# bibendovsky/oalsfxpp

Measured on AMD Instinct MI355X. Metric: Msamples/sec EAX reverb, 256-frame buffers, batch=4096; % HBM roofline, higher is better.
Workload: dtype f32

## Files before the change

oalsfxpp_amd/csrc/hip/reverb.hip:

```cpp
#include <float.h>

#include "common.hpp"
#include "wave_effects_body.hpp"

namespace oalsfx_hip {

namespace {

constexpr int kRow = 68;
constexpr int kGroups = 3;
constexpr int kSteadyGroups = 6;
constexpr int kRngFloats = OALSFX_RV_MAX_UPDATE;

namespace ut {
enum {
    TAP4 = 0,
    LO = 24,
    BMASK = 44,
    FEED4 = 49,
    CR_R = 50, CR_RF = 51,
    ECOEF = 52, ELCOEF = 56,
    MISC = 60,
    LPB = 64, HPB = 68,
    TL0 = 72, TL1 = 76, TH0 = 80, TH1 = 84,
// ... 558 lines not shown
        __hip_atomic_fetch_add(ctx.fault, 1u, __ATOMIC_RELAXED, __HIP_MEMORY_SCOPE_SYSTEM);
    }
    }
    stamp();
    const bool sf = SF && go && first && (flags & kFilterInside) != 0 && has_filter;
    float* const sfmisc = sh.sf_misc[SF ? wib : 0];
    auto sfrow = [&](int stage, int r) -> float* { return sh.sf_rows[SF ? wib : 0][SF ? stage * kSfRows + r : 0]; };
    if constexpr (SF) {
        if (lane == 0) sh.sf_all[wib] = sf ? 1 : 0;
        if (sf) {
            const oalsfx_source_params& SGp = ctx.source[inst];
            const oalsfx_source_state& SGs = ctx.source_state[inst];
            if (lane < 2) {
                const oalsfx_send_params& sp = lane == 0 ? SGp.direct : SGp.aux[slot];
                float* t = sfmisc + sfm::TAB + 12 * lane;
                t[0] = sp.lp.b0; t[1] = sp.lp.b1; t[2] = sp.lp.b2; t[3] = sp.hp.b0; t[4] = sp.hp.b1; t[5] = sp.hp.b2;
                t[6] = sp.lp.a1; t[7] = sp.lp.a2; t[8] = sp.hp.a1; t[9] = sp.hp.a2;
                const bool enabled = lane == 0 || sp.out_channels != 0;
                reinterpret_cast<int*>(t)[10] = enabled ? (((sp.filter_type & OALSFX_AF_LOW_PASS) ? 1 : 0) | ((sp.filter_type & OALSFX_AF_HIGH_PASS) ? 2 : 0) | 4) : 0;
            }
            if (lane < kSfRows) {
                const int sd = lane / CH, c = lane % CH, at = sd ? 1 + slot : 0;
                const oalsfx_hist_t lp = SGs.lp[at][c], hp = SGs.hp[at][c];
                float* h = sfmisc + sfm::HIST + 6 * lane;
                h[0] = lp.x[0]; h[1] = lp.x[1]; h[2] = lp.y[0]; h[3] = lp.y[1]; h[4] = hp.y[0]; h[5] = hp.y[1];
            }
        }
    }
    const bool filtered = !sf && (flags & kFiltered) != 0 && has_filter;
    const float* src = ctx.raw_src + static_cast<size_t>(inst) * ctx.io_stride;
    const float* wsrc = src;
    if (filtered) {
        src = ctx.src + static_cast<size_t>(inst) * ctx.src_stride;
        wsrc = ctx.wet_src + static_cast<size_t>(inst) * ctx.src_stride;
    }
    float* dst = ctx.dst + static_cast<size_t>(inst) * ctx.io_stride;
    float* mixbuf = ctx.mixbuf ? ctx.mixbuf + static_cast<size_t>(inst) * nch * OALSFX_MAX_CHUNK : nullptr;
    const float b2a = 0.288675134595F;

    v4f n_e = {0, 0, 0, 0}, n_a = n_e, n_el = n_e, n_lt = n_e, n_la = n_e, n_ll = n_e;
    float n_in0 = 0.0F, n_in1 = 0.0F;
    float n_inv[MC ? 8 : 1] = {};
    float n_w0 = 0.0F, n_w1 = 0.0F;
    float n_wv[MC ? 8 : 1] = {};
    auto tapbase = [&](int tile) -> int { return (XF && fc0 < OALSFX_RV_FADE_SAMPLES && fc0 + (tile << 6) >= OALSFX_RV_FADE_SAMPLES) ? kTapN : static_cast<int>(ut::TAP4); };
    auto load4 = [&](unsigned t4x, int group, auto ring, int base = ut::TAP4) -> v4f {
        constexpr int r = decltype(ring)::value;
        const v4u d = *reinterpret_cast<const v4u*>(utu + base + 4 * group);
        const v4u lo = *reinterpret_cast<const v4u*>(utu + ut::LO + 4 * r);
        const unsigned bm = utu[ut::BMASK + r];
        v4f v;
        v.x = ld_ring<r>(slab_b, ((t4x - d.x) & bm) | lo.x);
        v.y = ld_ring<r>(slab_b, ((t4x - d.y) & bm) | lo.y);
        v.z = ld_ring<r>(slab_b, ((t4x - d.z) & bm) | lo.z);
        v.w = ld_ring<r>(slab_b, ((t4x - d.w) & bm) | lo.w);
        return v;
    };
    constexpr bool AW = FP && !HY && !MD && !ST && !MC && !XF;
    v4f w_e = {0, 0, 0, 0}, w_el = w_e, w_lt = w_e, w_ll = w_e;
    auto load4w = [&](unsigned tile4, int group, auto ring) -> v4f {
        constexpr int r = decltype(ring)::value;
        const v4u d = *reinterpret_cast<const v4u*>(utu + ut::TAP4 + 4 * group);
        const v4u lo = *reinterpret_cast<const v4u*>(utu + ut::LO + 4 * r);
        const unsigned bm = utu[ut::BMASK + r];
        const unsigned l4 = 256u + 4u * static_cast<unsigned>(lane);
        v4f v;
        v.x = ld_ring<r>(slab_b, ((((tile4 - d.x) & ~255u) + l4) & bm) | lo.x);
        v.y = ld_ring<r>(slab_b, ((((tile4 - d.y) & ~255u) + l4) & bm) | lo.y);
        v.z = ld_ring<r>(slab_b, ((((tile4 - d.z) & ~255u) + l4) & bm) | lo.z);
        v.w = ld_ring<r>(slab_b, ((((tile4 - d.w) & ~255u) + l4) & bm) | lo.w);
        return v;
    };
    auto rotate4 = [&](const v4f& before, const v4f& last, unsigned tile4, int group) -> v4f {
        const v4u d = *reinterpret_cast<const v4u*>(utu + ut::TAP4 + 4 * group);
        auto one = [&](float b, float l, unsigned dj) -> float {
            const int k = static_cast<int>(((tile4 - dj) & 255u) >> 2);
            const float merged = lane >= k ? b : l;
            return __uint_as_float(static_cast<unsigned>(__builtin_amdgcn_ds_bpermute(((lane + k) & 63) << 2, static_cast<int>(__float_as_uint(merged)))));
        };
        v4f v;
        v.x = one(before.x, last.x, d.x); v.y = one(before.y, last.y, d.y); v.z = one(before.z, last.z, d.z); v.w = one(before.w, last.w, d.w);
        return v;
    };
    auto strow = [&](int k) -> float* { return utf + ut::SIZE + k * kRow; };
    float* modrow = utf + ut::SIZE;
    int mod_pos = v_modidx;
    auto next_mod_delays = [&](int samples_or_64) -> int {
        const int samples = RG ? samples_or_64 : 64;
        if (lane == 0) {
            float r = mod_f;
            const float depth = mod_depth, coeff = mod_coeff;
            for (int i = 0; i < samples; ++i) {
                r = lerpf(r, depth, coeff);
                modrow[i] = r;
            }
        }
        wave_sync();
        const float fv = modrow[lane];
        mod_f = modrow[samples - 1];
        wave_sync();
        int index;
        if (!RG && v_modrange >= 64) {
            index = mod_pos + lane;
            if (index >= v_modrange) index -= v_modrange;
            mod_pos += 64;
            if (mod_pos >= v_modrange) mod_pos -= v_modrange;
        } else {
            index = (mod_pos + lane) % v_modrange;
            mod_pos += 64;
        }
        const float sinus = glibc_sinf(6.28318530717958647692F * index / v_modrange);
        return lround_away(fv * sinus);
    };
    int md_next = 0, md_cur = 0;
    auto mb_buffer = [&](int pos) -> int {
        const int tile = __builtin_amdgcn_readfirstlane(pos) >> 6;
        return __builtin_amdgcn_readfirstlane(tile / (mbt->frames >> 6));
    };
    auto issue_input = [&](int posx) {
        const int px = min(posx, frames - 1);
        if (MC) {
#pragma unroll
            for (int c = 0; c < 8; ++c)
                if (c < nch) n_inv[MC ? c : 0] = src[static_cast<size_t>(px) * nch + c];
            if (filtered) {
#pragma unroll
                for (int c = 0; c < 8; ++c)
                    if (c < nch) n_wv[MC ? c : 0] = wsrc[static_cast<size_t>(px) * nch + c];
            }
        } else if (CH == 2) {
            const float2 v = *reinterpret_cast<const float2*>(src + static_cast<size_t>(px) * 2);
            n_in0 = v.x; n_in1 = v.y;
            if (filtered) {
                const float2 u = *reinterpret_cast<const float2*>(wsrc + static_cast<size_t>(px) * 2);
                n_w0 = u.x; n_w1 = u.y;
            }
        } else {
            n_in0 = src[px];
            if (filtered) n_w0 = wsrc[px];
        }
    };
    auto issue_taps_a = [&](unsigned t4x, int base) {
        if (AW) n_e = load4w(t4x - 4u * static_cast<unsigned>(lane), 0, RingId<OALSFX_RV_MAIN>{});
        else if (!HY || !(late_mask & 1u)) n_e = load4(t4x, 0, RingId<OALSFX_RV_MAIN>{}, base);
        if (!HY || !(late_mask & 2u)) n_a = load4(t4x, 1, RingId<OALSFX_RV_EARLY_AP>{}, base);
    };
    auto issue_taps_b = [&](unsigned t4x, int base) {
        if (AW) {
            const unsigned tile4 = t4x - 4u * static_cast<unsigned>(lane);
            n_el = load4w(tile4, 2, RingId<OALSFX_RV_EARLY_LINE>{});
            n_lt = load4w(tile4, 3, RingId<OALSFX_RV_MAIN>{});
            n_ll = load4w(tile4, 5, RingId<OALSFX_RV_LATE_LINE>{});
            return;
        }
        if (!HY || !(late_mask & 4u)) n_el = load4(t4x, 2, RingId<OALSFX_RV_EARLY_LINE>{}, base);
        if (!HY || !(late_mask & 8u)) n_lt = load4(t4x, 3, RingId<OALSFX_RV_MAIN>{}, base);
        if (!HY || !(late_mask & 32u)) n_ll = load4(MD ? t4x - 4u * static_cast<unsigned>(md_next) : t4x, 5, RingId<OALSFX_RV_LATE_LINE>{}, base);
    };
    auto issue_taps_c = [&](unsigned t4x, int base) {
        if (!HY || !(late_mask & 16u)) n_la = load4(t4x, 4, RingId<OALSFX_RV_LATE_AP>{}, base);
    };
    auto store4 = [&](unsigned p4, auto ring, float v0, float v1, float v2, float v3) {
        constexpr int r = decltype(ring)::value;
        const v4u lo = *reinterpret_cast<const v4u*>(utu + ut::LO + 4 * r);
        const unsigned wp = p4 & utu[ut::BMASK + r];
        st_ring<r>(slab_b, wp | lo.x, v0); st_ring<r>(slab_b, wp | lo.y, v1); st_ring<r>(slab_b, wp | lo.z, v2); st_ring<r>(slab_b, wp | lo.w, v3);
    };
    static_assert(CR == 0 || (AW && !SF), "line-aligned stores: the plain FP builds");
    auto cr_lane_before = [&](unsigned r) -> int { return ((lane - static_cast<int>(r)) & 63) << 2; };
    auto cr_rot = [&](int from4, float v) -> float { return __uint_as_float(static_cast<unsigned>(__builtin_amdgcn_ds_bpermute(from4, static_cast<int>(__float_as_uint(v))))); };
    auto carry_store = [&](unsigned tile4, auto ring, unsigned r, const v4f& rot, const v4f& before, bool head, bool tail, int L) {
        constexpr int rg = decltype(ring)::value;
        const v4u lo = *reinterpret_cast<const v4u*>(utu + ut::LO + 4 * rg);
        const unsigned bm = utu[ut::BMASK + rg];
        const bool held = lane < static_cast<int>(r);
        const int rl = static_cast<int>(r) + (RG ? L : 64);
        const unsigned at = tile4 - 4u * r + 4u * static_cast<unsigned>(lane);
        if (!(head && held) && (!RG || lane < rl)) {
            const unsigned wp = at & bm;
            st_ring<rg>(slab_b, wp | lo.x, held ? before.x : rot.x); st_ring<rg>(slab_b, wp | lo.y, held ? before.y : rot.y);
            st_ring<rg>(slab_b, wp | lo.z, held ? before.z : rot.z); st_ring<rg>(slab_b, wp | lo.w, held ? before.w : rot.w);
        }
        if (tail && (RG ? lane < rl - 64 : held)) {
            const unsigned wp = (at + 256u) & bm;
            st_ring<rg>(slab_b, wp | lo.x, rot.x); st_ring<rg>(slab_b, wp | lo.y, rot.y); st_ring<rg>(slab_b, wp | lo.z, rot.z); st_ring<rg>(slab_b, wp | lo.w, rot.w);
        }
    };
    auto cr_tail = [&](int site) -> v4f* { return reinterpret_cast<v4f*>(&sh.cr_tails[CR == 2 ? wib : 0][CR == 2 ? site : 0][lane & 31][0]); };
    auto carry_store_lds = [&](unsigned tile4, auto ring, int site, const v4f& rot, bool head, bool tail, int L) {
        v4f* t = cr_tail(site);
        const unsigned r = utu[ut::CR_R];
        const v4f before = *t;
        carry_store(tile4, ring, r, rot, before, head, tail, L);
        if (lane < static_cast<int>(r)) *t = rot;
    };
    v4f cr_feed = {0, 0, 0, 0};
    const int cw = (lane >> 2) & (NW - 1), cc = lane & 3;
    float* crowI0 = lds_all[cw] + (0 * 4 + cc) * kRow;
    float* crowI1 = lds_all[cw] + (1 * 4 + cc) * kRow;
    float* crowI2 = lds_all[cw] + (2 * 4 + cc) * kRow;
    float* crowL1 = lds_all[cw] + (4 * 4 + cc) * kRow;
    float* crowL2 = lds_all[cw] + (5 * 4 + cc) * kRow;
    float* cdat = chain_all[cw][cc];

    if (CR != 0 && go) {
        if (lane == 0) {
            utu[ut::CR_R] = static_cast<unsigned>(offset) & 31u;
            utu[ut::CR_RF] = (static_cast<unsigned>(offset) - (utu[ut::FEED4] >> 2)) & 31u;
        }
        wave_sync();
    }
    stamp();
    if (go) {
        if (FP && !(flags & kFiltered)) { n_in0 = early_in0; n_in1 = early_in1; }
        else issue_input(lane);
        if (AW) w_e = load4w((static_cast<unsigned>(offset) << 2) - 256u, 0, RingId<OALSFX_RV_MAIN>{});
        issue_taps_a(static_cast<unsigned>(offset + lane) << 2, tapbase(0));
    }
    stamp();
    lds_barrier();
    stamp();
    bool any_go = false;
    bool any_eax = false;
    bool any_sf = false;
#pragma unroll
    for (int k = 0; k < NW; ++k) { any_go |= go_all[k] != 0; any_eax |= eax_all[k] != 0; if (SF) any_sf |= sh.sf_all[k] != 0; }
    const bool chain_on = (lane < 4 * NW) && go_all[cw] != 0;
    const bool chain2_on = chain_on && eax_all[cw] != 0;
    const int duty = (wib - group) & (NW - 1);

    const int tiles = any_go ? (RG ? (frames + 63) >> 6 : frames >> 6) : 0;
    float o0 = 0.0F, o1 = 0.0F;
    float outv[MC ? 8 : 1] = {};
    int fc = fc0, blk_start = 0, blk_end = 0, blk_counter = 1;
    float g_step = 0.0F, g_run = 0.0F;
    bool g_ramp = false;
    unsigned long long ramp_mask = 0ULL;
    auto grow = [&](int q) -> float* { return q < 12 ? rowL(q >> 2, q & 3) + 4 : utf + ut::SIZE + (2 + q - 12) * kRow + 4; };
    constexpr bool EH = FP && !SF && !ST;
    auto hand_back = [&]() {
        if (go) {
            if (lane < 4) {
                const float* ch = chain_all[wib][lane];
                S.lp[lane].x[0] = ch[coop::LPX0]; S.lp[lane].x[1] = ch[coop::LPX1];
                S.lp[lane].y[0] = ch[coop::LPY0]; S.lp[lane].y[1] = ch[coop::LPY1];
                if (eax) {
                    S.hp[lane].x[0] = ch[coop::LPY0]; S.hp[lane].x[1] = ch[coop::LPY1];
                    S.hp[lane].y[0] = ch[coop::HPY0]; S.hp[lane].y[1] = ch[coop::HPY1];
                }
                S.t60[lane][0][0] = ch[coop::T60X]; S.t60[lane][0][1] = ch[coop::T60O1];
                S.t60[lane][1][0] = ch[coop::T60O1]; S.t60[lane][1][1] = ch[coop::T60O2];
            }
            if (lane == 0) {
                S.mod_index = static_cast<int>((static_cast<long long>(v_modidx) + frames) % v_modrange);
                S.offset = offset + frames;
                if (MD && mod_on) S.mod_filter = mod_f;
            }
            if (XF && xf_active) {
                if (q_valid) {
                    if (q_stage) S.late_cur_gain[q_line][q_chan] = g_cur;
                    else S.early_cur_gain[q_line][q_chan] = g_cur;
                }
                const bool fade_over = fc >= OALSFX_RV_FADE_SAMPLES;
                if (fc0 < OALSFX_RV_FADE_SAMPLES && fade_over && lane < 24) (&S.cur_early_tap[0])[lane] = static_cast<int32_t>(utu[kTapN + lane] >> 2);
                if (lane == 0) {
                    S.fade_count = fc;
                    S.mod_range = v_modrange;
                    SS.seen_seq = SP.update_seq;
                }
                if (ctx.exact) {
                    const unsigned level = gains_rest_level(q_valid, g_cur, g_tgt);
                    if (lane == 0) ctx.exact[sidx] = fade_over ? level : 0u;
                }
            }
            if (SF && sf) {
                if (lane < kSfRows) {
                    const int sd = lane / CH, c = lane % CH, at = sd ? 1 + slot : 0;
                    if (reinterpret_cast<const int*>(sfmisc + sfm::TAB + 12 * sd)[10] & 4) {
                        const float* h = sfmisc + sfm::HIST + 6 * lane;
                        oalsfx_source_state& SGs = ctx.source_state[inst];
                        oalsfx_hist_t lp, hp;
                        lp.x[0] = h[0]; lp.x[1] = h[1]; lp.y[0] = h[2]; lp.y[1] = h[3];
                        hp.x[0] = h[2]; hp.x[1] = h[3]; hp.y[0] = h[4]; hp.y[1] = h[5];
                        SGs.lp[at][c] = lp;
                        SGs.hp[at][c] = hp;
                    }
                }
            } else if (FP && !RG) {
                if (first && !filtered && lane < nch)
                    send_history_follow_values(ctx, inst, lane, send_mask, lane == 0 ? hist_new[0] : hist_new[CH - 1], lane == 0 ? hist_old[0] : hist_old[CH - 1]);
            } else if (first && !filtered && lane < nch) send_history_follow(ctx, inst, lane, nch, frames, src);
        }
        if constexpr (FP) {
            if (go) {
                if (lane == 0) {
                    miscu[hot::M_EPOCH] = epoch_now;
                    miscu[hot::M_OFFSET] = static_cast<unsigned>(offset + frames);
                    miscu[hot::M_MOD_F] = __float_as_uint(mod_f);
                    miscu[hot::M_MOD_INDEX] = static_cast<unsigned>((static_cast<long long>(v_modidx) + frames) % v_modrange);
                    miscu[hot::M_MOD_ON] = (MD && ((mod_depth != 0.0F) || (mod_f != 0.0F))) ? 1u : 0u;
                }
                wave_sync();
                v4u* rec = reinterpret_cast<v4u*>(ctx.hot + sidx * hot::SIZE);
                if (lane >= 48) rec[lane] = *reinterpret_cast<const v4u*>(miscu + 4 * (lane - 48));
                else if (lane >= 32) rec[lane] = *reinterpret_cast<const v4u*>(&chain_all[wib][0][0] + 4 * (lane - 32));
                else if (!hit) rec[lane] = *reinterpret_cast<const v4u*>(utu + 4 * lane);
            }
        }
    };
    for (int it = (SF && any_sf) ? -1 : 0; it <= tiles && tiles > 0; ++it) {
        const int ta = it, tb = it - 1, tc = it + 1;
        const bool has_a = ta >= 0 && ta < tiles, has_b = tb >= 0, has_c = SF && tc < tiles;
        const int pos_a = (ta << 6) + lane, pos_b = (tb << 6) + lane;
        const int La = RG ? min(64, frames - (ta << 6)) : 64;
        const int Lb = RG ? min(64, frames - (tb << 6)) : 64;
        const bool act = RG ? lane < Lb : true;
        const unsigned t4 = static_cast<unsigned>(offset + pos_b) << 2;
        const unsigned tile_b4 = static_cast<unsigned>(offset + (tb << 6)) << 2;
        const bool head_b = tb == 0, tail_b = tb == tiles - 1;
        float oa0 = 0.0F, oa1 = 0.0F;
        float outva[MC ? 8 : 1] = {};
        v4f p_e = n_e, p_a = n_a, p_el = n_el, p_lt = n_lt, p_la = n_la, p_ll = n_ll;
        if (AW && go && has_b) {
            const unsigned tile4 = static_cast<unsigned>(offset + (tb << 6)) << 2;
            p_e = rotate4(w_e, n_e, tile4, 0); p_el = rotate4(w_el, n_el, tile4, 2); p_lt = rotate4(w_lt, n_lt, tile4, 3); p_ll = rotate4(w_ll, n_ll, tile4, 5);
            w_e = n_e; w_el = n_el; w_lt = n_lt; w_ll = n_ll;
        }
        const int xg = eax ? 0 : 2;
        const bool xf_faded = XF && xf_active && has_b && fc0 + (tb << 6) < OALSFX_RV_FADE_SAMPLES;
        const float mu = static_cast<float>(fc0 + pos_b) * (1.0F / OALSFX_RV_FADE_SAMPLES);
        v4f q_e = {0, 0, 0, 0}, q_a = q_e, q_lt = q_e, q_el = q_e;
        auto mix4 = [&](v4f& a, const v4f& b) {
            a.x = lerpf(a.x, b.x, mu); a.y = lerpf(a.y, b.y, mu); a.z = lerpf(a.z, b.z, mu); a.w = lerpf(a.w, b.w, mu);
        };
        const int tb_base = tapbase(tb);

        if (go) {
            if (MD) {
                md_cur = md_next;
                if (mod_on && has_a) md_next = next_mod_delays(min(64, frames - (ta << 6)));
            }
            if (HY && has_b) {
                const int base = tapbase(tb);
                if (late_mask & 1u) p_e = load4(t4, 0, RingId<OALSFX_RV_MAIN>{}, base);
                if (late_mask & 2u) p_a = load4(t4, 1, RingId<OALSFX_RV_EARLY_AP>{}, base);
                if (late_mask & 4u) p_el = load4(t4, 2, RingId<OALSFX_RV_EARLY_LINE>{}, base);
                if (late_mask & 8u) p_lt = load4(t4, 3, RingId<OALSFX_RV_MAIN>{}, base);
                if (late_mask & 16u) p_la = load4(t4, 4, RingId<OALSFX_RV_LATE_AP>{}, base);
                if (late_mask & 32u) p_ll = load4(MD ? t4 - 4u * static_cast<unsigned>(md_cur) : t4, 5, RingId<OALSFX_RV_LATE_LINE>{}, base);
            }
            if (XF && xf_faded) {
                q_e = load4(t4, 0, RingId<OALSFX_RV_MAIN>{}, kTapN); q_a = load4(t4, 1, RingId<OALSFX_RV_EARLY_AP>{}, kTapN);
                q_lt = load4(t4, 3, RingId<OALSFX_RV_MAIN>{}, kTapN);
                q_el = load4(t4, 2, RingId<OALSFX_RV_EARLY_LINE>{}, kTapN);
                const v4f q_ll = load4(t4 - 4u * static_cast<unsigned>(md_cur), 5, RingId<OALSFX_RV_LATE_LINE>{}, kTapN);
                mix4(p_ll, q_ll);
            }
            if (has_a && it > 0) issue_taps_a(t4 + 256u, tapbase(ta));
            __builtin_amdgcn_sched_barrier(0);
        }
        v2f e01 = {0, 0}, e23 = {0, 0};
        float dg = 0.0F, ac = 0.0F, sx = 0.0F, sy = 0.0F;
        if (go && has_b) {
            if constexpr (CR == 2) {
                const int from = 4 + (cr_lane_before(utu[ut::CR_R]) >> 2);
                carry_store_lds(tile_b4, RingId<OALSFX_RV_MAIN>{}, 0, v4f{rowI(xg, 0)[from], rowI(xg, 1)[from], rowI(xg, 2)[from], rowI(xg, 3)[from]}, head_b, tail_b, Lb);
            } else if (act) store4(t4, RingId<OALSFX_RV_MAIN>{}, rowI(xg, 0)[4 + lane], rowI(xg, 1)[4 + lane], rowI(xg, 2)[4 + lane], rowI(xg, 3)[4 + lane]);
            wave_sync();
            const v4f misc = *reinterpret_cast<const v4f*>(utf + ut::MISC);
            dg = misc.x; ac = misc.y; sx = misc.z; sy = misc.w;
            const v4f ec = *reinterpret_cast<const v4f*>(utf + ut::ECOEF);
            const v4f elc = *reinterpret_cast<const v4f*>(utf + ut::ELCOEF);
            if (ST && (short_mask & 1u)) {
                auto hand_over = [&](v4f& v, int base) {
                    const v4u d = *reinterpret_cast<const v4u*>(utu + base);
                    const int e0 = static_cast<int>(d.x >> 2), e1 = static_cast<int>(d.y >> 2), e2 = static_cast<int>(d.z >> 2), e3 = static_cast<int>(d.w >> 2);
                    if (lane >= e0) v.x = rowI(xg, 0)[4 + lane - e0];
                    if (lane >= e1) v.y = rowI(xg, 1)[4 + lane - e1];
                    if (lane >= e2) v.z = rowI(xg, 2)[4 + lane - e2];
                    if (lane >= e3) v.w = rowI(xg, 3)[4 + lane - e3];
                };
                hand_over(p_e, XF ? tb_base : static_cast<int>(ut::TAP4));
                if (XF && xf_faded) hand_over(q_e, kTapN);
            }
            if (XF && xf_faded) mix4(p_e, q_e);
            if (ST && (short_mask & 2u)) {
                const v4u d = *reinterpret_cast<const v4u*>(utu + (XF ? tb_base : static_cast<int>(ut::TAP4)) + 4);
                const int o0x = static_cast<int>(d.x >> 2), o1x = static_cast<int>(d.y >> 2), o2x = static_cast<int>(d.z >> 2), o3x = static_cast<int>(d.w >> 2);
                int shortest_off = min(min(o0x, o1x), min(o2x, o3x));
                const v4u dn = *reinterpret_cast<const v4u*>(utu + (XF ? kTapN : static_cast<int>(ut::TAP4)) + 4);
                const int n0x = static_cast<int>(dn.x >> 2), n1x = static_cast<int>(dn.y >> 2), n2x = static_cast<int>(dn.z >> 2), n3x = static_cast<int>(dn.w >> 2);
                if (XF && xf_faded) shortest_off = min(shortest_off, min(min(n0x, n1x), min(n2x, n3x)));
                const int ahead = 63 / shortest_off;
                const v2f pf01 = v2f{p_e.x, p_e.y} * v2f{ec.x, ec.y};
                const v2f pf23 = v2f{p_e.z, p_e.w} * v2f{ec.z, ec.w};
                for (int k = 0; k < ahead; ++k) {
                    v4f a_now = p_a;
                    if (XF && xf_faded) mix4(a_now, q_a);
                    const v2f pv01 = v2f{a_now.x, a_now.y} - (ac * pf01);
                    const v2f pv23 = v2f{a_now.z, a_now.w} - (ac * pf23);
                    v2f pg01 = pf01 + (ac * pv01);
                    v2f pg23 = pf23 + (ac * pv23);
                    scatter2(pg01, pg23, sx, sy);
                    strow(0)[4 + lane] = pg01.x; strow(1)[4 + lane] = pg01.y; strow(2)[4 + lane] = pg23.x; strow(3)[4 + lane] = pg23.y;
                    wave_sync();
                    if (lane >= o0x) p_a.x = strow(0)[4 + lane - o0x];
                    if (lane >= o1x) p_a.y = strow(1)[4 + lane - o1x];
                    if (lane >= o2x) p_a.z = strow(2)[4 + lane - o2x];
                    if (lane >= o3x) p_a.w = strow(3)[4 + lane - o3x];
                    if (XF && xf_faded) {
                        if (lane >= n0x) q_a.x = strow(0)[4 + lane - n0x];
                        if (lane >= n1x) q_a.y = strow(1)[4 + lane - n1x];
                        if (lane >= n2x) q_a.z = strow(2)[4 + lane - n2x];
                        if (lane >= n3x) q_a.w = strow(3)[4 + lane - n3x];
                    }
                    wave_sync();
                }
            }
            if (XF && xf_faded) mix4(p_a, q_a);
            const v2f f01 = v2f{p_e.x, p_e.y} * v2f{ec.x, ec.y};
            const v2f f23 = v2f{p_e.z, p_e.w} * v2f{ec.z, ec.w};
            const v2f v01 = v2f{p_a.x, p_a.y} - (ac * f01);
            const v2f v23 = v2f{p_a.z, p_a.w} - (ac * f23);
            v2f g01 = f01 + (ac * v01);
            v2f g23 = f23 + (ac * v23);
            scatter2(g01, g23, sx, sy);
            if constexpr (CR == 2) {
                const int f4 = cr_lane_before(utu[ut::CR_R]);
                carry_store_lds(tile_b4, RingId<OALSFX_RV_EARLY_AP>{}, 1, v4f{cr_rot(f4, g01.x), cr_rot(f4, g01.y), cr_rot(f4, g23.x), cr_rot(f4, g23.y)}, head_b, tail_b, Lb);
                carry_store_lds(tile_b4, RingId<OALSFX_RV_EARLY_LINE>{}, 2, v4f{cr_rot(f4, v23.y), cr_rot(f4, v23.x), cr_rot(f4, v01.y), cr_rot(f4, v01.x)}, head_b, tail_b, Lb);
            } else if (act) {
                store4(t4, RingId<OALSFX_RV_EARLY_AP>{}, g01.x, g01.y, g23.x, g23.y);
                store4(t4, RingId<OALSFX_RV_EARLY_LINE>{}, v23.y, v23.x, v01.y, v01.x);
            }
            if (ST && (short_mask & 4u)) {
                strow(0)[4 + lane] = v23.y; strow(1)[4 + lane] = v23.x; strow(2)[4 + lane] = v01.y; strow(3)[4 + lane] = v01.x;
                wave_sync();
                auto hand_over = [&](v4f& v, int base) {
                    const v4u d = *reinterpret_cast<const v4u*>(utu + base + 8);
                    const int e0 = static_cast<int>(d.x >> 2), e1 = static_cast<int>(d.y >> 2), e2 = static_cast<int>(d.z >> 2), e3 = static_cast<int>(d.w >> 2);
// ... 22 lines not shown
                if (ST && (short_mask & 8u)) {
                    strow(4)[4 + lane] = r01.x; strow(5)[4 + lane] = r01.y; strow(6)[4 + lane] = r23.x; strow(7)[4 + lane] = r23.y;
                    wave_sync();
                    auto hand_over = [&](v4f& v, int base) {
                        const v4u d = *reinterpret_cast<const v4u*>(utu + base + 12);
                        const unsigned f4 = utu[ut::FEED4];
                        const int l0 = static_cast<int>((d.x - f4) >> 2), l1 = static_cast<int>((d.y - f4) >> 2), l2 = static_cast<int>((d.z - f4) >> 2),
                                  l3 = static_cast<int>((d.w - f4) >> 2);
                        if (lane >= l0) v.x = strow(4)[4 + lane - l0];
                        if (lane >= l1) v.y = strow(5)[4 + lane - l1];
                        if (lane >= l2) v.z = strow(6)[4 + lane - l2];
                        if (lane >= l3) v.w = strow(7)[4 + lane - l3];
                    };
                    hand_over(p_lt, XF ? tb_base : static_cast<int>(ut::TAP4));
                    if (XF && xf_faded) hand_over(q_lt, kTapN);
                }
            }
            if (XF && xf_faded) mix4(p_lt, q_lt);
            const v2f u01 = (v2f{p_lt.x, p_lt.y} * dg) + v2f{p_ll.x, p_ll.y};
            const v2f u23 = (v2f{p_lt.z, p_lt.w} * dg) + v2f{p_ll.z, p_ll.w};
            if (lane < 4) rowL(0, lane)[3] = chain_all[wib][lane][coop::T60X];
            rowL(0, 0)[4 + lane] = u01.x; rowL(0, 1)[4 + lane] = u01.y; rowL(0, 2)[4 + lane] = u23.x; rowL(0, 3)[4 + lane] = u23.y;
            wave_sync();
            {
                const v4f c0 = *reinterpret_cast<const v4f*>(utf + ut::TL0);
                const v4f c1 = *reinterpret_cast<const v4f*>(utf + ut::TL1);
                const float* xa = rowL(0, 0) + 4 + lane; const float* xb = rowL(0, 1) + 4 + lane;
                const float* xc = rowL(0, 2) + 4 + lane; const float* xd = rowL(0, 3) + 4 + lane;
                const v2f w01 = (v2f{c0.x, c0.y} * v2f{xa[0], xb[0]}) + (v2f{c1.x, c1.y} * v2f{xa[-1], xb[-1]});
                const v2f w23 = (v2f{c0.z, c0.w} * v2f{xc[0], xd[0]}) + (v2f{c1.z, c1.w} * v2f{xc[-1], xd[-1]});
                rowL(1, 0)[4 + lane] = w01.x; rowL(1, 1)[4 + lane] = w01.y; rowL(1, 2)[4 + lane] = w23.x; rowL(1, 3)[4 + lane] = w23.y;
            }
            if (lane < 4) chain_all[wib][lane][coop::T60X] = rowL(0, lane)[4 + Lb - 1];
        }
        if (go && has_a) {
            float in[2] = {n_in0, n_in1};
            float win[2] = {filtered ? n_w0 : n_in0, filtered ? n_w1 : n_in1};
            if (SF && sf) {
#pragma unroll
                for (int c = 0; c < (MC ? 0 : CH); ++c) { in[c] = sfrow(1, c)[4 + lane]; win[c] = sfrow(1, CH + c)[4 + lane]; }
            }
            float inv[MC ? 8 : 1], winv[MC ? 8 : 1];
#pragma unroll
            for (int c = 0; c < (MC ? 8 : 1); ++c) { inv[c] = n_inv[c]; winv[c] = filtered ? n_wv[c] : n_inv[c]; }
            if (!(SF && sf) && ta + 1 < tiles) {
                if constexpr (MB) {
                    const int k = mb_buffer(pos_a + 64);
                    src = mbt->src[k] + (static_cast<ptrdiff_t>(inst) * ctx.io_stride - static_cast<ptrdiff_t>(k) * mbt->frames * CH);
                }
                issue_input(pos_a + 64);
            }
            if (FP && !RG && !(SF && sf) && ta + 1 == tiles) {
#pragma unroll
                for (int c = 0; c < (MC ? 0 : CH); ++c) {
                    hist_new[c] = __uint_as_float(__builtin_amdgcn_readlane(__float_as_uint(in[c]), 63));
                    hist_old[c] = __uint_as_float(__builtin_amdgcn_readlane(__float_as_uint(in[c]), 62));
                }
            }
            float wet[4] = {0.0F, 0.0F, 0.0F, 0.0F};
            if (MC) {
#pragma unroll
                for (int c = 0; c < 8; ++c) {
                    if (c >= nch) continue;
                    if (first) {
#pragma unroll
                        for (int o = 0; o < 8; ++o)
                            if (aud_dir & (1ULL << (c * 8 + o))) outva[MC ? o : 0] += inv[MC ? c : 0] * utf[kMcBase + 64 + c * 8 + o];
                    }
#pragma unroll
                    for (int k = 0; k < 4; ++k)
                        if (aud_aux & (1ULL << (c * 4 + k))) wet[k] += winv[MC ? c : 0] * utf[kMcBase + 128 + c * 4 + k];
                }
                if (!first) {
#pragma unroll
                    for (int c = 0; c < 8; ++c)
                        if (c < nch) outva[MC ? c : 0] = mixbuf[c * OALSFX_MAX_CHUNK + pos_a];
                }
            } else if (!first) {
                oa0 = mixbuf[pos_a];
                if (CH == 2) oa1 = mixbuf[OALSFX_MAX_CHUNK + pos_a];
            } else {
                const v4f gd = *reinterpret_cast<const v4f*>(utf + ut::GDIR);
                const float g[4] = {gd.x, gd.y, gd.z, gd.w};
#pragma unroll
                for (int c = 0; c < (MC ? 0 : CH); ++c) {
                    if (aud_dir & (1u << (c * 2 + 0))) oa0 += in[c] * g[c * 2 + 0];
                    if (CH == 2 && (aud_dir & (1u << (c * 2 + 1)))) oa1 += in[c] * g[c * 2 + 1];
                }
            }
#pragma unroll
            for (int c = 0; c < (MC ? 0 : CH); ++c) {
                const v4f ga = *reinterpret_cast<const v4f*>(utf + ut::GAUX + 4 * c);
                const float g[4] = {ga.x, ga.y, ga.z, ga.w};
#pragma unroll
                for (int k = 0; k < 4; ++k)
                    if (aud_aux & (1u << (c * 4 + k))) wet[k] += win[c] * g[k];
            }
            v2f a01 = {0.0F, 0.0F}, a23 = {0.0F, 0.0F};
            a01 = a01 + wet[0] * v2f{b2a, b2a}; a01 = a01 + wet[1] * v2f{b2a, -b2a}; a01 = a01 + wet[2] * v2f{b2a, -b2a}; a01 = a01 + wet[3] * v2f{b2a, b2a};
            a23 = a23 + wet[0] * v2f{b2a, b2a}; a23 = a23 + wet[1] * v2f{b2a, -b2a}; a23 = a23 + wet[2] * v2f{-b2a, b2a}; a23 = a23 + wet[3] * v2f{-b2a, -b2a};
            if (lane < 4) {
                const float* ch = chain_all[wib][lane];
                rowI(0, lane)[3] = ch[coop::LPX0]; rowI(0, lane)[2] = ch[coop::LPX1];
            }
            rowI(0, 0)[4 + lane] = a01.x; rowI(0, 1)[4 + lane] = a01.y; rowI(0, 2)[4 + lane] = a23.x; rowI(0, 3)[4 + lane] = a23.y;
            wave_sync();
            {
                const v4f bq = *reinterpret_cast<const v4f*>(utf + ut::LPB);
                const float* xa = rowI(0, 0) + 4 + lane; const float* xb = rowI(0, 1) + 4 + lane;
                const float* xc = rowI(0, 2) + 4 + lane; const float* xd = rowI(0, 3) + 4 + lane;
                const v2f u01 = ((bq.x * v2f{xa[0], xb[0]}) + (bq.y * v2f{xa[-1], xb[-1]})) + (bq.z * v2f{xa[-2], xb[-2]});
                const v2f u23 = ((bq.x * v2f{xc[0], xd[0]}) + (bq.y * v2f{xc[-1], xd[-1]})) + (bq.z * v2f{xc[-2], xd[-2]});
                rowI(1, 0)[4 + lane] = u01.x; rowI(1, 1)[4 + lane] = u01.y; rowI(1, 2)[4 + lane] = u23.x; rowI(1, 3)[4 + lane] = u23.y;
            }
            if (lane < 4) {
                float* ch = chain_all[wib][lane];
                ch[coop::LPX1] = rowI(0, lane)[4 + La - 2]; ch[coop::LPX0] = rowI(0, lane)[4 + La - 1];
            }
        }
        if (SF && sf && has_c) {
            const float x[2] = {n_in0, n_in1};
            if (tc + 1 < tiles) issue_input(((tc + 1) << 6) + lane);
#pragma unroll
            for (int c = 0; c < (MC ? 0 : CH); ++c) {
                if (lane < 2) sfmisc[sfm::EDGE + 4 * c + lane] = x[c];
                if (lane >= 62) sfmisc[sfm::EDGE + 4 * c + lane - 60] = x[c];
                const float xm1 = __shfl_up(x[c], 1), xm2 = __shfl_up(x[c], 2);
#pragma unroll
                for (int sd = 0; sd < 2; ++sd) {
                    const float* t = sfmisc + sfm::TAB + 12 * sd;
                    const int mode = __builtin_amdgcn_readfirstlane(reinterpret_cast<const int*>(t)[10]);
                    if (!(mode & 4)) continue;
                    float v = x[c];
                    if ((mode & 1) && lane >= 2) v = (t[0] * x[c]) + (t[1] * xm1) + (t[2] * xm2);
                    sfrow(0, sd * CH + c)[4 + lane] = v;
                }
            }
        }
        if (go && has_a) {
            if (AW && ta == 0) {
                const unsigned before4 = (static_cast<unsigned>(offset) << 2) - 256u;
                w_el = load4w(before4, 2, RingId<OALSFX_RV_EARLY_LINE>{}); w_lt = load4w(before4, 3, RingId<OALSFX_RV_MAIN>{}); w_ll = load4w(before4, 5, RingId<OALSFX_RV_LATE_LINE>{});
            }
            issue_taps_b(static_cast<unsigned>(offset + pos_a) << 2, tapbase(ta));
            __builtin_amdgcn_sched_barrier(0);
        }
        stamp();
        lds_barrier();
        stamp();
        if (duty == ((NW == 2) ? 0 : 0 + ((NW > 4) ? (it & 1) * 4 : 0)) && chain_on && has_a) {
            __builtin_amdgcn_s_setprio(3);
            float y1 = cdat[coop::LPY0], y2 = cdat[coop::LPY1];
            const float h1 = y1, h2 = y2;
            if (!RG || La == 64) biquad_chain(crowI1, crowI2, 64, cdat[coop::LP_A1], cdat[coop::LP_A2], y1, y2);
            else biquad_chain(crowI1, crowI2, La, cdat[coop::LP_A1], cdat[coop::LP_A2], y1, y2);
            crowI2[3] = h1; crowI2[2] = h2;
            cdat[coop::LPY0] = y1; cdat[coop::LPY1] = y2;
            __builtin_amdgcn_s_setprio(0);
        }
        if (SF && any_sf && duty == 1 && has_c && lane < NW * kSfRows) {
            const int cwx = lane / kSfRows, rr = lane % kSfRows, sd = rr / CH, c = rr % CH;
            float* m = sh.sf_misc[SF ? cwx : 0];
            const float* t = m + sfm::TAB + 12 * sd;
            const int mode = sh.sf_all[cwx] ? reinterpret_cast<const int*>(t)[10] : 0;
            if (mode & 4) {
                float* h = m + sfm::HIST + 6 * rr;
                float* wrow = sh.sf_rows[SF ? cwx : 0][SF ? rr : 0];
                const float* e = m + sfm::EDGE + 4 * c;
                float y1 = h[2], y2 = h[3];
                if (mode & 1) {
                    const float x1 = h[0], x2 = h[1];
                    wrow[4] = (t[0] * e[0]) + (t[1] * x1) + (t[2] * x2);
                    wrow[5] = (t[0] * e[1]) + (t[1] * e[0]) + (t[2] * x1);
                }
                wrow[2] = y2; wrow[3] = y1;
                if (mode & 1) biquad_chain(wrow, wrow, 64, t[6], t[7], y1, y2);
                else { y1 = e[3]; y2 = e[2]; }
                h[0] = e[3]; h[1] = e[2]; h[2] = y1; h[3] = y2;
            }
        }
        if (duty == ((NW == 2) ? 0 : 2 + ((NW > 4) ? (it & 1) * 4 : 0)) && chain_on && has_b) {
            __builtin_amdgcn_s_setprio(3);
            float prev = cdat[coop::T60O1];
            const float before = prev;
            if (!RG || Lb == 64) first_order_chain(crowL1, crowL2, 0, 64, cdat[coop::T_L2], 1.0F, false, prev);
            else first_order_chain(crowL1, crowL2, 0, Lb, cdat[coop::T_L2], 1.0F, false, prev);
            crowL2[3] = before;
            cdat[coop::T60O1] = prev;
            __builtin_amdgcn_s_setprio(0);
        }
        stamp();
        lds_barrier();
        stamp();
        if (go && has_a) {
            issue_taps_c(static_cast<unsigned>(offset + pos_a) << 2, tapbase(ta));
            __builtin_amdgcn_sched_barrier(0);
        }
        if (SF && sf && has_c) {
#pragma unroll
            for (int sd = 0; sd < 2; ++sd) {
                const float* t = sfmisc + sfm::TAB + 12 * sd;
                const int mode = __builtin_amdgcn_readfirstlane(reinterpret_cast<const int*>(t)[10]);
                if (!(mode & 4)) continue;
#pragma unroll
                for (int c = 0; c < (MC ? 0 : CH); ++c) {
                    const float* y = sfrow(0, sd * CH + c) + 4 + lane;
                    float v = y[0];
                    if ((mode & 6) == 6) v = (t[3] * y[0]) + (t[4] * y[-1]) + (t[5] * y[-2]);
                    sfrow(1, sd * CH + c)[4 + lane] = v;
                }
            }
        }
        if (any_eax) {
            if (go && eax && has_a) {
                const v4f bq = *reinterpret_cast<const v4f*>(utf + ut::HPB);
                const float* xa = rowI(2, 0) + 4 + lane; const float* xb = rowI(2, 1) + 4 + lane;
                const float* xc = rowI(2, 2) + 4 + lane; const float* xd = rowI(2, 3) + 4 + lane;
                const v2f u01 = ((bq.x * v2f{xa[0], xb[0]}) + (bq.y * v2f{xa[-1], xb[-1]})) + (bq.z * v2f{xa[-2], xb[-2]});
                const v2f u23 = ((bq.x * v2f{xc[0], xd[0]}) + (bq.y * v2f{xc[-1], xd[-1]})) + (bq.z * v2f{xc[-2], xd[-2]});
                rowI(1, 0)[4 + lane] = u01.x; rowI(1, 1)[4 + lane] = u01.y; rowI(1, 2)[4 + lane] = u23.x; rowI(1, 3)[4 + lane] = u23.y;
            }
        }
        if (go && has_b) {
            const v4f c0 = *reinterpret_cast<const v4f*>(utf + ut::TH0);
            const v4f c1 = *reinterpret_cast<const v4f*>(utf + ut::TH1);
// ... 103 lines not shown
                if (!act) {
                } else if (last && ctx.turn_set != 0u) {
                    if ((nch & 1) == 0) {
#pragma unroll
                        for (int c = 0; c < 8; c += 2)
                            if (c < nch) {
                                const unsigned long long both = static_cast<unsigned long long>(__float_as_uint(outv[MC ? c : 0])) |
                                                                (static_cast<unsigned long long>(__float_as_uint(outv[MC ? c + 1 : 0])) << 32);
                                __hip_atomic_store(reinterpret_cast<unsigned long long*>(dst + static_cast<size_t>(pos_b) * nch + c), both, __ATOMIC_RELAXED, __HIP_MEMORY_SCOPE_AGENT);
                            }
                    } else {
                        const bool odd = (pos_b & 1) != 0;
                        float* frame = dst + static_cast<size_t>(pos_b) * nch;
#pragma unroll
                        for (int k = 0; k < 3; ++k) {
                            const float lo = odd ? outv[MC ? 2 * k + 1 : 0] : outv[MC ? 2 * k : 0];
                            const float hi = odd ? outv[MC ? 2 * k + 2 : 0] : outv[MC ? 2 * k + 1 : 0];
                            const int at = 2 * k + (odd ? 1 : 0);
                            if (at + 1 < nch) {
                                const unsigned long long both = static_cast<unsigned long long>(__float_as_uint(lo)) | (static_cast<unsigned long long>(__float_as_uint(hi)) << 32);
                                __hip_atomic_store(reinterpret_cast<unsigned long long*>(frame + at), both, __ATOMIC_RELAXED, __HIP_MEMORY_SCOPE_AGENT);
                            }
                        }
                        const int alone = odd ? 0 : nch - 1;
                        float v = outv[0];
#pragma unroll
                        for (int c = 1; c < 8; ++c)
                            if (MC && c == alone) v = outv[MC ? c : 0];
                        __hip_atomic_store(reinterpret_cast<unsigned*>(frame + alone), __float_as_uint(v), __ATOMIC_RELAXED, __HIP_MEMORY_SCOPE_AGENT);
                    }
                } else if (last) {
#pragma unroll
                    for (int c = 0; c < 8; ++c)
                        if (c < nch) dst[static_cast<size_t>(pos_b) * nch + c] = outv[MC ? c : 0];
                } else {
#pragma unroll
                    for (int c = 0; c < 8; ++c)
                        if (c < nch) mixbuf[c * OALSFX_MAX_CHUNK + pos_b] = outv[MC ? c : 0];
                }
            }
            if (XF && xf_active) {
                const int tpos = tb << 6;
                if (tpos == blk_end) {
                    blk_start = tpos;
                    int todo = min(frames - tpos, OALSFX_RV_MAX_UPDATE);
                    if (fc < OALSFX_RV_FADE_SAMPLES) todo = min(todo, OALSFX_RV_FADE_SAMPLES - fc);
                    blk_end = tpos + todo;
                    blk_counter = frames - tpos;
                    g_step = (g_tgt - g_cur) * (1.0F / static_cast<float>(blk_counter));
                    g_ramp = q_valid && (fabsf(g_step) > FLT_EPSILON);
                    ramp_mask = __ballot(g_ramp);
                    g_run = g_cur;
                }
                if (ramp_mask != 0ULL) {
                    if (g_ramp) {
                        float* gs = grow(lane);
                        for (int i = 0; i < 64; ++i) {
                            gs[i] = g_run;
                            g_run += g_step;
                        }
                    }
                    wave_sync();
                }
#pragma unroll
                for (int k = 0; k < 8; ++k) {
#pragma unroll
                    for (int c = 0; c < (MC ? 0 : CH); ++c) {
                        const int q = k * CH + c;
                        float& o = c == 0 ? o0 : o1;
                        if ((ramp_mask >> q) & 1ULL) {
                            o += data[k] * grow(q)[lane];
                        } else {
                            const float gq = __uint_as_float(__builtin_amdgcn_readlane(__float_as_uint(g_cur), q));
                            if (audible(gq)) o += data[k] * gq;
                        }
                    }
                }
                if (ramp_mask != 0ULL) wave_sync();
                if (tpos + 64 == blk_end) {
                    if (g_ramp) g_cur = (blk_end == frames) ? g_tgt : g_run;
                    if (fc < OALSFX_RV_FADE_SAMPLES) fc = min(fc + (blk_end - blk_start), OALSFX_RV_FADE_SAMPLES);
                }
            } else {
#pragma unroll
                for (int k = 0; k < (MC ? 0 : 8); k += 2) {
                    const v4f g = *reinterpret_cast<const v4f*>(utf + ut::GOUT + 2 * k);
                    if (aud_out & (1u << (2 * k + 0))) o0 += data[k] * g.x;
                    if (CH == 2 && (aud_out & (1u << (2 * k + 1)))) o1 += data[k] * g.y;
                    if (aud_out & (1u << (2 * k + 2))) o0 += data[k + 1] * g.z;
                    if (CH == 2 && (aud_out & (1u << (2 * k + 3)))) o1 += data[k + 1] * g.w;
                }
            }
            if (MC || !act) {
            } else if (last) {
                float* out = dst;
                int pos_o = pos_b;
                if constexpr (MB) {
                    const int k = mb_buffer(pos_b);
                    out = mbt->dst[k] + static_cast<size_t>(inst) * ctx.io_stride;
                    pos_o -= k * mbt->frames;
                }
                if (ctx.turn_set != 0u) {
                    if (CH == 2) {
                        const unsigned long long both = static_cast<unsigned long long>(__float_as_uint(o0)) | (static_cast<unsigned long long>(__float_as_uint(o1)) << 32);
                        __hip_atomic_store(reinterpret_cast<unsigned long long*>(out + static_cast<size_t>(pos_o) * 2), both, __ATOMIC_RELAXED, __HIP_MEMORY_SCOPE_AGENT);
                    } else __hip_atomic_store(reinterpret_cast<unsigned*>(out + pos_o), __float_as_uint(o0), __ATOMIC_RELAXED, __HIP_MEMORY_SCOPE_AGENT);
                } else if (CH == 2) {
                    *reinterpret_cast<float2*>(out + static_cast<size_t>(pos_o) * 2) = make_float2(o0, o1);
                } else out[pos_o] = o0;
            } else {
                mixbuf[pos_b] = o0;
                if (CH == 2) mixbuf[OALSFX_MAX_CHUNK + pos_b] = o1;
            }
            wave_sync();
        }
        o0 = oa0; o1 = oa1;
#pragma unroll
        for (int c = 0; c < (MC ? 8 : 1); ++c) outv[c] = outva[c];
        stamp();
    }

    if (!EH) hand_back();
    if constexpr (FP) {
    } else
    if (MC || ctx.progress != nullptr) {
        if (valid && lane == 0) ctx.progress[sidx] = go ? frames : 0;
        if (valid && lane == 0 && !go && w < ctx.no_follow_up && ctx.fault) __hip_atomic_fetch_add(ctx.fault, 1u, __ATOMIC_RELAXED, __HIP_MEMORY_SCOPE_SYSTEM);
    } else if constexpr (!MC) {
        if (valid && !go) {
            KernelCtx copy = ctx;
            reverb_general_call<CH>(&copy, slot, inst, flags & 0xFF, lds, lane);
        }
    }
    if (ctx.turn != nullptr && ctx.turn_set != 0u) {
        __builtin_amdgcn_fence(__ATOMIC_RELEASE, "workgroup");
        if (valid && lane == 0) {
            __hip_atomic_store(ctx.turn_cu2 + sidx, cu_before, __ATOMIC_RELAXED, __HIP_MEMORY_SCOPE_AGENT);
            __hip_atomic_store(ctx.turn_cu + sidx, this_cu(), __ATOMIC_RELAXED, __HIP_MEMORY_SCOPE_AGENT);
        }
        __builtin_amdgcn_s_waitcnt(0);
        if (valid && lane == 0) __hip_atomic_store(ctx.turn + sidx, ctx.turn_set, __ATOMIC_RELAXED, __HIP_MEMORY_SCOPE_AGENT);
    }
    stamp();
}

template <int CH, int NW, bool TL = false, bool HY = false, bool MD = false, bool ST = false, bool RG = false, bool FP = false, bool XF = false, bool NF = false, bool SF = false, int CR = 0>
__global__ __launch_bounds__(64 * NW, 4) void k_reverb_steady_coop(KernelCtx ctx, int slot, const int* __restrict__ list, int count, int flags)
{
    __shared__ SteadyShared<CH, NW, FP, MD, ST, SF, CR> sh;
    reverb_steady_group<CH, NW, TL, HY, MD, ST, RG, FP, XF, NF, SF, CR>(ctx, slot, list, count, flags, static_cast<int>(blockIdx.x), sh);
}

template <int CH, int NW, bool TL = false, bool HY = false, bool MD = false, bool ST = false, bool RG = false, bool FP = false, bool XF = false, bool NF = false, bool SF = false, int CR = 0>
__global__ __launch_bounds__(64 * NW, 4) void k_reverb_steady_coop_ep(KernelCtx ctx, int slot, const int* __restrict__ list, int count, int flags)
{
    __shared__ SteadyShared<CH, NW, FP, MD, ST, SF, CR> sh;
    reverb_steady_group<CH, NW, TL, HY, MD, ST, RG, FP, XF, NF, SF, CR>(ctx, slot, list, count, flags, static_cast<int>(blockIdx.x), sh);
    if constexpr (!(RG && CR == 2 && CH == 2)) OALSFX_EQUAL_PLACES();
}

struct SteadyKinds {
    int count[4];
    __host__ __device__ int groups(int k) const { return (count[k] + 3) >> 2; }
};

template <int CH, bool NF, bool SF, int CR = 0>
__global__ __launch_bounds__(256, 4) void k_reverb_steady_kinds(KernelCtx ctx, int slot, const int* __restrict__ list, SteadyKinds kinds, int flags)
{
    static_assert(!SF || CR == 0, "send filters inside and line-aligned stores: no LDS for both");
    union Shared {
        SteadyShared<CH, 4, true, false, false, SF, CR> lean;
        SteadyShared<CH, 4, true, true, true> general;
        SteadyShared<CH, 4, false, true, true> believed;
// ... 889 lines not shown
```

Baseline: 28070.

## Keep aligned-window tap cursors in registers with scalar-base loads and ballot rotates

For aligned-window variants without the SF path, the code now precomputes a per-lane window cursor (tap delay, ring low bits and mask) once and advances it with a bit-field insert each tile. It no longer recomputes ring addresses from the tap table on every load. Loads use a scalar base read from that cursor plus a per-lane offset, and rotates use an inverse-ballot select. Separately, the audible masks are forced into scalar registers so the gain branches stay uniform. The aim is to cut VALU address arithmetic and LDS table reads in the hot loop. In exchange it relies on wave-uniform assumptions and inline asm constraints, and adds readlane traffic.

Result: faster. 29020 (median of 5 runs) (+3.4%).

```diff
diff --git a/oalsfxpp_amd/csrc/hip/reverb.hip b/oalsfxpp_amd/csrc/hip/reverb.hip
--- a/oalsfxpp_amd/csrc/hip/reverb.hip
+++ b/oalsfxpp_amd/csrc/hip/reverb.hip
@@ -664,6 +664,53 @@
         v.x = one(before.x, last.x, d.x); v.y = one(before.y, last.y, d.y); v.z = one(before.z, last.z, d.z); v.w = one(before.w, last.w, d.w);
         return v;
     };
+    static_assert(kPlainMinTap >= 64, "aligned windows: a ring shorter than a window would wrap inside it");
+    constexpr bool LS = AW && !SF;
+    auto in_loop = [&](unsigned long long mask) -> unsigned long long {
+        if constexpr (LS) {
+            unsigned m = __builtin_amdgcn_readfirstlane(static_cast<unsigned>(mask));
+            asm volatile("" : "+s"(m));
+            return m;
+        } else return mask;
+    };
+    unsigned aw_cur = 0u, aw_bm = 0u;
+    const unsigned lane4 = 4u * static_cast<unsigned>(lane);
+    auto aw_init = [&](unsigned before4) {
+        const int j = lane & 15, g = j >> 2, c = j & 3;
+        const int grp = (0x5320 >> (4 * g)) & 15;
+        const int r = (((OALSFX_RV_LATE_LINE << 12) | (OALSFX_RV_MAIN << 8) | (OALSFX_RV_EARLY_LINE << 4) | OALSFX_RV_MAIN) >> (4 * g)) & 15;
+        const unsigned d = utu[ut::TAP4 + 4 * grp + c], lo = utu[ut::LO + 4 * r + c];
+        aw_bm = utu[ut::BMASK + r];
+        aw_cur = (((((before4 - d) & ~255u) + 256u) & aw_bm) | lo) | ((before4 - d) & 255u);
+    };
+    auto aw_moved = [&](unsigned cur, unsigned by) -> unsigned {
+        unsigned moved;
+        asm("v_bfi_b32 %0, %1, %2, %3" : "=v"(moved) : "v"(aw_bm), "v"(cur + by), "v"(cur));
+        return moved;
+    };
+    auto aw_load4 = [&](unsigned cur, auto gsel, auto ring) -> v4f {
+        constexpr int r = decltype(ring)::value;
+        constexpr int G = decltype(gsel)::value;
+        unsigned l4 = lane4;
+        asm volatile("" : "+v"(l4));
+        auto one = [&](int j) -> float {
+            unsigned long long base = reinterpret_cast<unsigned long long>(slab_b) + (static_cast<unsigned>(__builtin_amdgcn_readlane(static_cast<int>(cur), j)) & ~255u);
+            asm("" : "+s"(base));
+            return ld_ring<r>(reinterpret_cast<const GlobalBytes*>(base), l4);
+        };
+        return v4f{one(4 * G + 0), one(4 * G + 1), one(4 * G + 2), one(4 * G + 3)};
+    };
+    auto aw_rotate4 = [&](const v4f& before, const v4f& last, auto gsel) -> v4f {
+        constexpr int G = decltype(gsel)::value;
+        auto one = [&](float b, float l, int j) -> float {
+            const unsigned k4 = static_cast<unsigned>(__builtin_amdgcn_readlane(static_cast<int>(aw_cur), j)) & 255u;
+            const float merged = __builtin_amdgcn_inverse_ballot_w64(~0ULL << (k4 >> 2)) ? b : l;
+            return __uint_as_float(static_cast<unsigned>(__builtin_amdgcn_ds_bpermute(static_cast<int>(lane4 + k4), static_cast<int>(__float_as_uint(merged)))));
+        };
+        v4f v;
+        v.x = one(before.x, last.x, 4 * G + 0); v.y = one(before.y, last.y, 4 * G + 1); v.z = one(before.z, last.z, 4 * G + 2); v.w = one(before.w, last.w, 4 * G + 3);
+        return v;
+    };
     auto strow = [&](int k) -> float* { return utf + ut::SIZE + k * kRow; };
     float* modrow = utf + ut::SIZE;
     int mod_pos = v_modidx;
@@ -723,12 +770,18 @@
         }
     };
     auto issue_taps_a = [&](unsigned t4x, int base) {
-        if (AW) n_e = load4w(t4x - 4u * static_cast<unsigned>(lane), 0, RingId<OALSFX_RV_MAIN>{});
+        if constexpr (LS) n_e = aw_load4(aw_cur, RingId<0>{}, RingId<OALSFX_RV_MAIN>{});
+        else if (AW) n_e = load4w(t4x - 4u * static_cast<unsigned>(lane), 0, RingId<OALSFX_RV_MAIN>{});
         else if (!HY || !(late_mask & 1u)) n_e = load4(t4x, 0, RingId<OALSFX_RV_MAIN>{}, base);
         if (!HY || !(late_mask & 2u)) n_a = load4(t4x, 1, RingId<OALSFX_RV_EARLY_AP>{}, base);
     };
     auto issue_taps_b = [&](unsigned t4x, int base) {
-        if (AW) {
+        if constexpr (LS) {
+            n_el = aw_load4(aw_cur, RingId<1>{}, RingId<OALSFX_RV_EARLY_LINE>{});
+            n_lt = aw_load4(aw_cur, RingId<2>{}, RingId<OALSFX_RV_MAIN>{});
+            n_ll = aw_load4(aw_cur, RingId<3>{}, RingId<OALSFX_RV_LATE_LINE>{});
+            return;
+        } else if (AW) {
             const unsigned tile4 = t4x - 4u * static_cast<unsigned>(lane);
             n_el = load4w(tile4, 2, RingId<OALSFX_RV_EARLY_LINE>{});
             n_lt = load4w(tile4, 3, RingId<OALSFX_RV_MAIN>{});
@@ -796,7 +849,11 @@
     if (go) {
         if (FP && !(flags & kFiltered)) { n_in0 = early_in0; n_in1 = early_in1; }
         else issue_input(lane);
-        if (AW) w_e = load4w((static_cast<unsigned>(offset) << 2) - 256u, 0, RingId<OALSFX_RV_MAIN>{});
+        if constexpr (LS) {
+            aw_init((static_cast<unsigned>(offset) << 2) - 256u);
+            w_e = aw_load4(aw_cur, RingId<0>{}, RingId<OALSFX_RV_MAIN>{});
+            aw_cur = aw_moved(aw_cur, 256u);
+        } else if (AW) w_e = load4w((static_cast<unsigned>(offset) << 2) - 256u, 0, RingId<OALSFX_RV_MAIN>{});
         issue_taps_a(static_cast<unsigned>(offset + lane) << 2, tapbase(0));
     }
     stamp();
@@ -905,7 +962,11 @@
         v4f p_e = n_e, p_a = n_a, p_el = n_el, p_lt = n_lt, p_la = n_la, p_ll = n_ll;
         if (AW && go && has_b) {
             const unsigned tile4 = static_cast<unsigned>(offset + (tb << 6)) << 2;
+            if constexpr (LS) {
+                p_e = aw_rotate4(w_e, n_e, RingId<0>{}); p_el = aw_rotate4(w_el, n_el, RingId<1>{}); p_lt = aw_rotate4(w_lt, n_lt, RingId<2>{}); p_ll = aw_rotate4(w_ll, n_ll, RingId<3>{});
+            } else {
             p_e = rotate4(w_e, n_e, tile4, 0); p_el = rotate4(w_el, n_el, tile4, 2); p_lt = rotate4(w_lt, n_lt, tile4, 3); p_ll = rotate4(w_ll, n_ll, tile4, 5);
+            }
             w_e = n_e; w_el = n_el; w_lt = n_lt; w_ll = n_ll;
         }
         const int xg = eax ? 0 : 2;
@@ -938,6 +999,7 @@
                 const v4f q_ll = load4(t4 - 4u * static_cast<unsigned>(md_cur), 5, RingId<OALSFX_RV_LATE_LINE>{}, kTapN);
                 mix4(p_ll, q_ll);
             }
+            if (LS && has_a && it > 0) aw_cur = aw_moved(aw_cur, 256u);
             if (has_a && it > 0) issue_taps_a(t4 + 256u, tapbase(ta));
             __builtin_amdgcn_sched_barrier(0);
         }
@@ -1126,19 +1188,21 @@
             } else {
                 const v4f gd = *reinterpret_cast<const v4f*>(utf + ut::GDIR);
                 const float g[4] = {gd.x, gd.y, gd.z, gd.w};
+                const unsigned long long dir = in_loop(aud_dir);
 #pragma unroll
                 for (int c = 0; c < (MC ? 0 : CH); ++c) {
-                    if (aud_dir & (1u << (c * 2 + 0))) oa0 += in[c] * g[c * 2 + 0];
-                    if (CH == 2 && (aud_dir & (1u << (c * 2 + 1)))) oa1 += in[c] * g[c * 2 + 1];
-                }
-            }
+                    if (dir & (1u << (c * 2 + 0))) oa0 += in[c] * g[c * 2 + 0];
+                    if (CH == 2 && (dir & (1u << (c * 2 + 1)))) oa1 += in[c] * g[c * 2 + 1];
+                }
+            }
+            const unsigned long long aux = in_loop(aud_aux);
 #pragma unroll
             for (int c = 0; c < (MC ? 0 : CH); ++c) {
                 const v4f ga = *reinterpret_cast<const v4f*>(utf + ut::GAUX + 4 * c);
                 const float g[4] = {ga.x, ga.y, ga.z, ga.w};
 #pragma unroll
                 for (int k = 0; k < 4; ++k)
-                    if (aud_aux & (1u << (c * 4 + k))) wet[k] += win[c] * g[k];
+                    if (aux & (1u << (c * 4 + k))) wet[k] += win[c] * g[k];
             }
             v2f a01 = {0.0F, 0.0F}, a23 = {0.0F, 0.0F};
             a01 = a01 + wet[0] * v2f{b2a, b2a}; a01 = a01 + wet[1] * v2f{b2a, -b2a}; a01 = a01 + wet[2] * v2f{b2a, -b2a}; a01 = a01 + wet[3] * v2f{b2a, b2a};
@@ -1184,7 +1248,12 @@
         if (go && has_a) {
             if (AW && ta == 0) {
                 const unsigned before4 = (static_cast<unsigned>(offset) << 2) - 256u;
+                if constexpr (LS) {
+                    const unsigned before = aw_moved(aw_cur, 0u - 256u);
+                    w_el = aw_load4(before, RingId<1>{}, RingId<OALSFX_RV_EARLY_LINE>{}); w_lt = aw_load4(before, RingId<2>{}, RingId<OALSFX_RV_MAIN>{}); w_ll = aw_load4(before, RingId<3>{}, RingId<OALSFX_RV_LATE_LINE>{});
+                } else {
                 w_el = load4w(before4, 2, RingId<OALSFX_RV_EARLY_LINE>{}); w_lt = load4w(before4, 3, RingId<OALSFX_RV_MAIN>{}); w_ll = load4w(before4, 5, RingId<OALSFX_RV_LATE_LINE>{});
+                }
             }
             issue_taps_b(static_cast<unsigned>(offset + pos_a) << 2, tapbase(ta));
             __builtin_amdgcn_sched_barrier(0);
@@ -1454,13 +1523,14 @@
                     if (fc < OALSFX_RV_FADE_SAMPLES) fc = min(fc + (blk_end - blk_start), OALSFX_RV_FADE_SAMPLES);
                 }
             } else {
+                const unsigned long long out = in_loop(aud_out);
 #pragma unroll
                 for (int k = 0; k < (MC ? 0 : 8); k += 2) {
                     const v4f g = *reinterpret_cast<const v4f*>(utf + ut::GOUT + 2 * k);
-                    if (aud_out & (1u << (2 * k + 0))) o0 += data[k] * g.x;
-                    if (CH == 2 && (aud_out & (1u << (2 * k + 1)))) o1 += data[k] * g.y;
-                    if (aud_out & (1u << (2 * k + 2))) o0 += data[k + 1] * g.z;
-                    if (CH == 2 && (aud_out & (1u << (2 * k + 3)))) o1 += data[k + 1] * g.w;
+                    if (out & (1u << (2 * k + 0))) o0 += data[k] * g.x;
+                    if (CH == 2 && (out & (1u << (2 * k + 1)))) o1 += data[k] * g.y;
+                    if (out & (1u << (2 * k + 2))) o0 += data[k + 1] * g.z;
+                    if (CH == 2 && (out & (1u << (2 * k + 3)))) o1 += data[k + 1] * g.w;
                 }
             }
             if (MC || !act) {
```
